# BaileyMeche/FM-ReturnPrediction

Hardware: AMD Instinct MI355X
Metric: firm-month rows/sec (and % HBM roofline) for full FM pass at 1/2/4/8 MI355X (higher is better)
Workload: dtype f64; 1 GPU; C3+C4 full pass per GPU: 600 months x 5000 firms x 15 chars; winsorize 1/99 -> NYSE universes -> M1/M2/M3 x 3 universes + Fig-1 x 2 -> NW(4) -> rolling 120/60 -> lagged-rolling forecasts + predictive-slope FM; months_per_gpu=600, firms=5000, chars=15, problems_per_month=11, global_months=600, seed=1, parallelism=month-sharded x1

## Files before the change

fm-returnprediction_amd/csrc/fm_solve.hip:

```cpp
#include <math.h>

#include <type_traits>

#include "fm_common.h"

FM_PROBE_BUFFER(solve)

namespace fm {
namespace {

constexpr int VT = 256;
constexpr int VNW = VT / WAVE;
constexpr int MAXB_LDS = 8192;
constexpr int64_t SCAN_GRID = 1024;
constexpr double CHOL_REL = 1e-9;
constexpr double EIG_REL = 1e-12;
constexpr double REFIT_REL = 1e-6;

template <int MD>
struct WaveScratch {
    double A[MD * MD];
    double V[MD * MD];
    double sxy[MD], sdiag[MD], mu[MD], b[MD];
};

template <int MD>
__device__ void jacobi_pinv(double* A, double* V, int K, const double* sxy, const double* mur, double* b) {
    for (int i = 0; i < K; ++i)
        for (int j = 0; j < K; ++j) V[i * MD + j] = i == j ? 1.0 : 0.0;
    double frob = 0.0;
    for (int i = 0; i < K; ++i)
        for (int j = 0; j < K; ++j) frob += A[i * MD + j] * A[i * MD + j];
    for (int sweep = 0; sweep < 80; ++sweep) {
        double off = 0.0;
        for (int p = 0; p < K; ++p)
            for (int q = p + 1; q < K; ++q) off += A[p * MD + q] * A[p * MD + q];
        if (off <= 1e-34 * frob) break;
        for (int p = 0; p < K; ++p) {
            for (int q = p + 1; q < K; ++q) {
                const double apq = A[p * MD + q];
                if (apq == 0.0) continue;
                const double theta = (A[q * MD + q] - A[p * MD + p]) / (2.0 * apq);
                const double t = (theta >= 0.0 ? 1.0 : -1.0) / (fabs(theta) + sqrt(theta * theta + 1.0));
                const double c = 1.0 / sqrt(t * t + 1.0), s = t * c;
                for (int k = 0; k < K; ++k) {
                    const double akp = A[k * MD + p], akq = A[k * MD + q];
                    A[k * MD + p] = c * akp - s * akq;
                    A[k * MD + q] = s * akp + c * akq;
                }
                for (int k = 0; k < K; ++k) {
                    const double apk = A[p * MD + k], aqk = A[q * MD + k];
                    A[p * MD + k] = c * apk - s * aqk;
                    A[q * MD + k] = s * apk + c * aqk;
                }
                A[p * MD + q] = 0.0;
                A[q * MD + p] = 0.0;
                for (int k = 0; k < K; ++k) {
                    const double vkp = V[k * MD + p], vkq = V[k * MD + q];
                    V[k * MD + p] = c * vkp - s * vkq;
                    V[k * MD + q] = s * vkp + c * vkq;
                }
            }
        }
    }
    double lmax = 0.0;
    for (int i = 0; i < K; ++i) lmax = fmax(lmax, fabs(A[i * MD + i]));
    for (int j = 0; j < K; ++j) b[j] = 0.0;
    for (int i = 0; i < K; ++i) {
        const double l = A[i * MD + i];
        if (!(l > EIG_REL * lmax)) continue;
        double proj = 0.0;
        for (int k = 0; k < K; ++k) proj += V[k * MD + i] * sxy[k];
        proj /= l;
        for (int j = 0; j < K; ++j) b[j] += proj * V[j * MD + i];
    }
    double b0 = mur[K], den = 1.0;
    for (int j = 0; j < K; ++j) b0 -= b[j] * mur[j];
    for (int i = 0; i < K; ++i) {
        if (A[i * MD + i] > EIG_REL * lmax) continue;
        double wi = 0.0;
        for (int k = 0; k < K; ++k) wi += V[k * MD + i] * mur[k];
        den += wi * wi;
    }
    if (!(den > 1.0) || !isfinite(b0)) return;
    for (int i = 0; i < K; ++i) {
        if (A[i * MD + i] > EIG_REL * lmax) continue;
        double wi = 0.0;
        for (int k = 0; k < K; ++k) wi += V[k * MD + i] * mur[k];
        const double t = b0 * wi / den;
        for (int j = 0; j < K; ++j) b[j] += t * V[j * MD + i];
    }
}

__device__ __forceinline__ double readlane_f64(double v, int l) {
    return __longlong_as_double((long long)readlane_u64((uint64_t)__double_as_longlong(v), l));
}

template <int NT>
__device__ __forceinline__ void sum_partials(const double* partial, int c0, int c1, int n, double* bs) {
    constexpr int BCH = 8;
    const int tid = threadIdx.x;
    for (int e0 = tid; e0 < n; e0 += NT * BCH) {
        double acc[BCH];
#pragma unroll
        for (int k = 0; k < BCH; ++k) acc[k] = 0.0;
        for (int c = c0; c < c1; ++c) {
            const double* pc = partial + (int64_t)c * n;
#pragma unroll
            for (int k = 0; k < BCH; ++k) {
                const int e = e0 + k * NT;
                acc[k] += pc[e < n ? e : n - 1];
            }
        }
#pragma unroll
        for (int k = 0; k < BCH; ++k) {
            const int e = e0 + k * NT;
            if (e < n) bs[e] = acc[k];
        }
    }
}

template <int MD>
__global__ __launch_bounds__(VT) void solve_kernel(fm_solve_args a) {
    extern __shared__ double bs[];
    __shared__ WaveScratch<MD> ws_all[VNW];
    const int s = blockIdx.x;
    const int tid = threadIdx.x, lane = tid & (WAVE - 1);
    const int w = __builtin_amdgcn_readfirstlane(tid / WAVE);
    const int zw = a.zw, zz = zw * (zw + 1) / 2;
    const int nl = a.nlevels, npat = a.npatterns, nb = npat * nl;
    const int c0 = a.seg_chunk_off[s], c1 = a.seg_chunk_off[s + 1];
    sum_partials<VT>(a.partial, c0, c1, nb * zz, bs);
    __syncthreads();
    for (int e = tid; e < npat * zz; e += VT) {
        const int pid = e / zz, f = e - pid * zz;
        double* b0 = bs + (int64_t)pid * nl * zz + f;
        double run = b0[(nl - 1) * zz];
        for (int l = nl - 2; l >= 0; --l) {
            run += b0[l * zz];
            b0[l * zz] = run;
        }
    }
    __syncthreads();
    WaveScratch<MD>& ws = ws_all[w];
    const int rs = a.pmax + 2;
    constexpr int PKW = MD * (MD + 1) / 2;
    constexpr int EPL = (PKW + WAVE - 1) / WAVE;
    for (int p = w; p < a.nprob; p += VNW) {
        const int m = a.prob_model[p], u = a.prob_level[p], nz = a.prob_nz[p];
        const int* zi = a.prob_z + p * 32;
        const int K = nz - 2, K1 = K + 1;
        int off[EPL], dst[EPL], dsw[EPL];
        double acc[EPL];
#pragma unroll
        for (int t = 0; t < EPL; ++t) {
            const int e = lane + WAVE * t;
            int i = 0, rem = e;
            while (i < nz && rem >= nz - i) {
                rem -= nz - i;
                ++i;
            }
            const bool in = i < nz;
            const int j = in ? i + rem : 0;
            const int zr = in ? zi[i] : 0, zc = in ? zi[j] : 0;
            const int r = zr < zc ? zr : zc, c = zr < zc ? zc : zr;
            off[t] = in ? r * zw - (r * (r - 1)) / 2 + (c - r) : 0;
            dst[t] = in ? i * MD + j : -1;
            dsw[t] = in ? j * MD + i : -1;
            acc[t] = 0.0;
        }
        for (int q = 0; q < npat; ++q) {
            if (!((a.pattern_models[q] >> m) & 1u)) continue;
            const double* bq = bs + (q * nl + u) * zz;
#pragma unroll
            for (int t = 0; t < EPL; ++t) acc[t] += bq[off[t]];
        }
#pragma unroll
        for (int t = 0; t < EPL; ++t)
            if (dst[t] >= 0) {
                ws.V[dst[t]] = acc[t];
                ws.V[dsw[t]] = acc[t];
            }
        wave_sync();
        const double* Gp = ws.V;
        const int zl = lane < K1 ? zi[1 + lane] : 0;
        const int li = lane < K1 ? 1 + lane : 0;
        const double n = Gp[0];
        const double g0 = lane < K1 ? Gp[li] : 0.0;
        const double gdiag = lane < K1 ? Gp[li * MD + li] : 0.0;
        const int64_t ro = ((int64_t)s * a.nprob + p) * rs;
        uint32_t st = 0;
        if (__ballot(lane < K && isinf(gdiag)) != 0) st |= FM_ST_INF_IN_X;
        if (__ballot(lane == K && isinf(gdiag)) != 0) st |= FM_ST_INF_IN_Y;
        if (a.gram_flags) st |= a.gram_flags[(int64_t)s * a.nmodels + m] & (FM_ST_INF_IN_X | FM_ST_INF_IN_Y);
        if (!(n >= (double)(K + 1))) {
            for (int k = lane; k < rs; k += WAVE) a.rec[ro + k] = k == a.pmax + 1 ? n : NAN;
            if (lane == 0) a.status[(int64_t)s * a.nprob + p] = FM_ST_SKIPPED;
            continue;
        }
        double row[MD];
        double sii = 0.0, sxy = 0.0;
#pragma unroll
        for (int j = 0; j < MD; ++j) {
            row[j] = 0.0;
            if (j < K1) {
                const double v = lane < K1 ? Gp[li * MD + 1 + j] - g0 * Gp[1 + j] / n : 0.0;
                row[j] = v;
                if (j == lane) sii = v;
                if (j == K) sxy = v;
            }
        }
        const double mu = g0 / n;
        if (a.moments) {
            double* mo = a.moments + ((int64_t)s * a.nprob + p) * a.mom_stride;
            if (lane == 0) mo[0] = n;
            if (lane < K1) {
                mo[1 + lane] = mu;
#pragma unroll
                for (int j = 0; j < MD; ++j)
                    if (j < K1) mo[1 + K1 + lane * K1 + j] = row[j];
            }
        }
        if ((a.prob_flags[p] & 1) != 0) {
            if (__ballot(lane < K && !(sii > 1e-10 * gdiag)) != 0) st |= FM_ST_CONST_SUSPECT;
        }
        const double syy = readlane_f64(sii, K);
        bool ok = true;
#pragma unroll
        for (int k = 0; k < MD - 1; ++k) {
            if (ok && k < K) {
                const double orig = readlane_f64(sii, k);
                const double piv = readlane_f64(row[k], k);
                if (!(piv > REFIT_REL * orig)) st |= FM_ST_REFIT;
                if (!(orig > 0.0) || !(piv > CHOL_REL * orig)) {
                    ok = false;
                } else {
                    const double lkk = sqrt(piv);
                    const double rinv = 1.0 / lkk;
                    const double lik = row[k] * rinv;
#pragma unroll
                    for (int j = k + 1; j < MD; ++j) {
                        if (j <= K) {
                            const double sj = readlane_f64(row[j], k) * rinv;
                            row[j] -= lik * sj;
                        }
                    }
                    row[k] = lane == k ? lkk : lik;
                }
            }
        }
        double bi = 0.0;
        if (ok) {
            double* T = ws.A;
#pragma unroll
            for (int j = 0; j < MD; ++j)
                if (lane < K1) T[lane * MD + j] = row[j];
            wave_sync();
            double col[MD];
#pragma unroll
            for (int r = 0; r < MD; ++r) col[r] = lane < MD ? T[r * MD + (lane & (MD - 1))] : 0.0;
            double t = lane < K ? T[K * MD + lane] : 0.0;
#pragma unroll
            for (int j = MD - 2; j >= 0; --j) {
                if (j < K) {
                    const double bj = readlane_f64(t, j) / readlane_f64(col[j], j);
                    if (lane == j) t = bj;
                    else if (lane < j) t -= col[j] * bj;
                }
            }
            bi = lane < K ? t : 0.0;
            wave_sync();
        } else {
            st |= FM_ST_RANK_DEF | FM_ST_REFIT;
#pragma unroll
            for (int j = 0; j < MD; ++j)
                if (j < K && lane < K) ws.A[lane * MD + j] = Gp[li * MD + 1 + j] - g0 * Gp[1 + j] / n;
            if (lane < K) ws.sxy[lane] = sxy;
            if (lane < K1) ws.mu[lane] = mu + (a.add_back ? a.add_back[(int64_t)(zl - 1) * a.nseg + s] : 0.0);
            wave_sync();
            if (lane == 0) jacobi_pinv<MD>(ws.A, ws.V, K, ws.sxy, ws.mu, ws.b);
            wave_sync();
            bi = lane < K ? ws.b[lane] : 0.0;
            wave_sync();
        }
        double t_sxy = lane < K ? bi * sxy : 0.0;
        double t_mu = lane < K ? bi * mu : 0.0;
        double t_ab = 0.0;
        if (a.add_back && lane < K) t_ab = bi * a.add_back[(int64_t)(zl - 1) * a.nseg + s];
        t_sxy = wave_sum(t_sxy);
        t_mu = wave_sum(t_mu);
        t_ab = wave_sum(t_ab);
        const double r2 = 1.0 - (syy - t_sxy) / syy;
        double icpt = readlane_f64(mu, K) - t_mu;
        if (a.add_back) icpt += a.add_back[(int64_t)(zi[K + 1] - 1) * a.nseg + s] - t_ab;
        const double bsh = __shfl(bi, lane > 0 ? lane - 1 : 0, WAVE);
        for (int k = lane; k < rs; k += WAVE) {
            double v = NAN;
            if (k == 0) v = icpt;
            else if (k <= K) v = bsh;
            else if (k == a.pmax) v = r2;
            else if (k == a.pmax + 1) v = n;
            a.rec[ro + k] = v;
        }
        if (lane == 0) a.status[(int64_t)s * a.nprob + p] = st | FM_ST_FITTED;
    }
}

template <class CA>
struct FixCtx {
    CA cols; int64_t stride; const int64_t* seg_off; int nseg;
    const double *lo, *hi;
    const double *shift, *inv_scale, *add_back;
    const uint8_t* level;
    int nprob; const int32_t *prob_level, *prob_z, *prob_nz;
    const double* moments; int mom_stride;
    int pmax; double* rec; uint32_t* status;
    int check_const;
};

template <class CA>
__host__ __device__ __forceinline__ FixCtx<CA> fix_ctx(const fm_solve_args& a, CA cols) {
    FixCtx<CA> fx{};
    fx.check_const = a.fix_check_const;
    fx.cols = cols, fx.stride = a.fix_stride, fx.seg_off = a.fix_seg_off, fx.nseg = a.nseg;
    fx.lo = a.fix_lo, fx.hi = a.fix_hi;
    fx.shift = a.fix_shift, fx.inv_scale = a.fix_inv_scale, fx.add_back = a.add_back;
    fx.level = a.fix_level;
    fx.nprob = a.nprob, fx.prob_level = a.prob_level, fx.prob_z = a.prob_z, fx.prob_nz = a.prob_nz;
    fx.moments = a.moments, fx.mom_stride = a.mom_stride;
    fx.pmax = a.pmax, fx.rec = a.rec, fx.status = a.status;
    return fx;
}

template <int NT = VT, class CA = F64Cols>
__device__ __forceinline__ void const_pair(int s, int p, uint64_t* red, const FixCtx<CA>& fx) {
    const int nz = fx.prob_nz[p], K = nz - 2, u = fx.prob_level[p];
    const int* zi = fx.prob_z + p * 32;
    const int64_t r0 = fx.seg_off[s], r1 = fx.seg_off[s + 1];
    bool any_const = false;
    for (int j = 0; j < K; ++j) {
        const int cx = zi[1 + j] - 1;
        uint64_t kmin = SENT, kmax = 0;
        bool allnz = true;
        for (int64_t r = r0 + threadIdx.x; r < r1; r += NT) {
            if (fx.level && (int)fx.level[r] < u) continue;
            bool ok = true;
            double xv = 0.0;
            for (int q = 1; q < nz; ++q) {
                const int c = zi[q] - 1;
                double x = fx.cols[(int64_t)c * fx.stride + r];
                if (fx.lo) {
                    const double l = fx.lo[(int64_t)c * fx.nseg + s], h = fx.hi[(int64_t)c * fx.nseg + s];
                    if (x < l) x = l;
                    if (x > h) x = h;
                }
                if (isnan(x)) ok = false;
                if (c == cx) xv = x;
            }
            if (!ok) continue;
            const uint64_t k = dkey(xv == 0.0 ? 0.0 : xv);
            kmin = k < kmin ? k : kmin;
            kmax = k > kmax ? k : kmax;
            if (xv == 0.0) allnz = false;
        }
        kmin = block_min_u64<NT / WAVE>(kmin, red);
        kmax = block_max_u64<NT / WAVE>(kmax, red);
        const int nzr = block_sum<NT / WAVE>(allnz ? 0 : 1, (int*)red);
        if (kmin != SENT && kmin == kmax && nzr == 0) any_const = true;
    }
    if (threadIdx.x == 0 && any_const) fx.status[(int64_t)s * fx.nprob + p] |= FM_ST_CONST_COL;
}

struct InfySmem {
    double Lm[32 * 32];
    double mu[32], xb[32];
    unsigned bits[32];
    int okf;
};

template <int NT = VT, int NC = 32, class CA = F64Cols>
__device__ __forceinline__ void infy_pair(int s, int p, InfySmem& sm, const FixCtx<CA>& fx) {
    double* Lm = sm.Lm;
    double* mu = sm.mu;
    double* xb = sm.xb;
    unsigned* bits = sm.bits;
    int& okf = sm.okf;
    const int nz = fx.prob_nz[p], K = nz - 2, K1 = K + 1, u = fx.prob_level[p];
    const int* zi = fx.prob_z + p * 32;
    const double* mo = fx.moments + ((int64_t)s * fx.nprob + p) * fx.mom_stride;
    const double n = mo[0];
    for (int e = threadIdx.x; e < K * K; e += NT) Lm[(e / K) * 32 + e % K] = mo[1 + K1 + (e / K) * K1 + e % K];
    if (threadIdx.x < K1) mu[threadIdx.x] = mo[1 + threadIdx.x];
    if (threadIdx.x < 32) bits[threadIdx.x] = 0u;
    __syncthreads();
    if (threadIdx.x < K) {
        const int c = zi[1 + threadIdx.x] - 1;
        xb[threadIdx.x] = mu[threadIdx.x] + (fx.add_back ? fx.add_back[(int64_t)c * fx.nseg + s] : 0.0);
    }
    if (threadIdx.x == 0) {
        int ok = 1;
        for (int k = 0; k < K && ok; ++k) {
            double d = Lm[k * 32 + k];
            for (int j = 0; j < k; ++j) d -= Lm[k * 32 + j] * Lm[k * 32 + j];
            if (!(d > 0.0)) { ok = 0; break; }
            d = sqrt(d);
            Lm[k * 32 + k] = d;
            for (int i = k + 1; i < K; ++i) {
                double t = Lm[i * 32 + k];
                for (int j = 0; j < k; ++j) t -= Lm[i * 32 + j] * Lm[k * 32 + j];
                Lm[i * 32 + k] = t / d;
            }
        }
        okf = ok;
    }
    __syncthreads();
    if (!okf) return;
    const int64_t r0 = fx.seg_off[s], r1 = fx.seg_off[s + 1];
    if constexpr (NC <= 16) {
        for (int64_t r = r0 + threadIdx.x; r < r1; r += NT) {
            if (fx.level && (int)fx.level[r] < u) continue;
            int zo = 0;
            asm volatile("" : "+v"(zo));
            double d[NC];
            double y = 0.0;
            bool valid = true;
#pragma unroll
            for (int q = 1; q <= NC; ++q) {
                if (q < nz) {
                    const int c = zi[q] - 1;
                    double x = fx.cols[(int64_t)c * fx.stride + r];
                    if (fx.lo) {
                        const double l = fx.lo[(int64_t)c * fx.nseg + s], h = fx.hi[(int64_t)c * fx.nseg + s];
                        if (x < l) x = l;
                        if (x > h) x = h;
                    }
                    if (isnan(x)) valid = false;
                    if (q == nz - 1) {
                        y = x;
                    } else {
                        if (fx.shift) x -= fx.shift[(int64_t)c * fx.nseg + s];
                        if (fx.inv_scale) x *= fx.inv_scale[(int64_t)c * fx.nseg + s];
                        d[q - 1] = x - mu[q - 1 + zo];
                    }
                }
            }
            if (!valid || !isinf(y)) continue;
#pragma unroll
            for (int i = 0; i < NC; ++i) {
                if (i < K) {
                    double t = d[i];
#pragma unroll
                    for (int j = 0; j < i; ++j) t -= Lm[i * 32 + j + zo] * d[j];
                    d[i] = t / Lm[i * 32 + i + zo];
                }
            }
#pragma unroll
            for (int i = NC - 1; i >= 0; --i) {
                if (i < K) {
                    double t = d[i];
#pragma unroll
                    for (int j = i + 1; j < NC; ++j)
                        if (j < K) t -= Lm[j * 32 + i + zo] * d[j];
                    d[i] = t / Lm[i * 32 + i + zo];
                }
            }
            double c0 = 1.0 / n;
#pragma unroll
            for (int j = 0; j < NC; ++j)
                if (j < K) c0 -= xb[j + zo] * d[j];
#pragma unroll
            for (int j = 0; j <= NC; ++j) {
                if (j <= K) {
                    const double term = (j == 0 ? c0 : d[j == 0 ? 0 : j - 1]) * y;
                    const unsigned b = isnan(term) ? 4u : (term > 0.0 ? 1u : 2u);
                    atomicOr(&bits[j], b);
                }
            }
        }
    } else
    for (int64_t r = r0 + threadIdx.x; r < r1; r += NT) {
        if (fx.level && (int)fx.level[r] < u) continue;
        double v[32];
        bool valid = true;
        for (int q = 1; q < nz; ++q) {
            const int c = zi[q] - 1;
            double x = fx.cols[(int64_t)c * fx.stride + r];
            if (fx.lo) {
                const double l = fx.lo[(int64_t)c * fx.nseg + s], h = fx.hi[(int64_t)c * fx.nseg + s];
                if (x < l) x = l;
                if (x > h) x = h;
            }
            if (isnan(x)) valid = false;
            v[q - 1] = x;
        }
        if (!valid || !isinf(v[K])) continue;
        const double y = v[K];
        double d[32];
        for (int j = 0; j < K; ++j) {
            const int c = zi[1 + j] - 1;
            double x = v[j];
            if (fx.shift) x -= fx.shift[(int64_t)c * fx.nseg + s];
            if (fx.inv_scale) x *= fx.inv_scale[(int64_t)c * fx.nseg + s];
            d[j] = x - mu[j];
        }
        for (int i = 0; i < K; ++i) {
            double t = d[i];
            for (int j = 0; j < i; ++j) t -= Lm[i * 32 + j] * d[j];
            d[i] = t / Lm[i * 32 + i];
        }
        for (int i = K - 1; i >= 0; --i) {
            double t = d[i];
            for (int j = i + 1; j < K; ++j) t -= Lm[j * 32 + i] * d[j];
            d[i] = t / Lm[i * 32 + i];
        }
        double c0 = 1.0 / n;
        for (int j = 0; j < K; ++j) c0 -= xb[j] * d[j];
        for (int j = 0; j <= K; ++j) {
            const double term = (j == 0 ? c0 : d[j - 1]) * y;
            const unsigned b = isnan(term) ? 4u : (term > 0.0 ? 1u : 2u);
            atomicOr(&bits[j], b);
        }
    }
    __syncthreads();
    const int64_t ro = ((int64_t)s * fx.nprob + p) * (fx.pmax + 2);
    if (threadIdx.x <= K) {
        const unsigned b = bits[threadIdx.x];
        if (b != 0u) {
            double val = NAN;
            if (!(b & 4u) && b != 3u) val = (b & 1u) ? INFINITY : -INFINITY;
            fx.rec[ro + threadIdx.x] = val;
        }
    }
    if (threadIdx.x == 0) fx.rec[ro + fx.pmax] = NAN;
}

constexpr double SVD_REL = 1e-13;

__device__ __forceinline__ double wave_sum_dpp(double v) {
    v += xor_lanes_f64(v, 1);
    v += xor_lanes_f64(v, 2);
    v += xor_lanes_f64(v, 4);
    v += xor_lanes_f64(v, 8);
    v += xor_lanes_f64(v, 16);
    v += xor_lanes_f64(v, 32);
    return v;
}

template <int NC, int NW = VNW>
struct RefitSmem {
    double R[NW][NC][NC + 1];
    double Ac[NC][NC + 1];
    double Vc[NC][NC + 1];
    double bv[NC];
};

template <int NC>
__device__ __forceinline__ void hh_absorb(double (&a)[NC], double (*R)[NC + 1], int nzc) {
    const int lane = lane_id();
    static_for<0, NC>([&](auto kc) {
        constexpr int k = decltype(kc)::value;
        if (k < nzc) {
            const double ss = wave_sum_dpp(a[k] * a[k]);
            if (ss != 0.0) {
                const double alpha = R[k][k];
                const double nrm = sqrt(alpha * alpha + ss);
                const double beta = alpha > 0.0 ? -nrm : nrm;
                const double v0 = alpha - beta;
                const double tau = -v0 / beta;
                const double vl = a[k] / v0;
                double w[NC];
                static_for<k + 1, NC>([&](auto jc) {
                    constexpr int j = decltype(jc)::value;
                    w[j] = vl * a[j];
                });
                static_for<k + 1, NC>([&](auto jc) {
                    constexpr int j = decltype(jc)::value;
                    w[j] = wave_sum_dpp(w[j]) + R[k][j];
                });
                static_for<k + 1, NC>([&](auto jc) {
                    constexpr int j = decltype(jc)::value;
                    a[j] -= (tau * w[j]) * vl;
                });
                __builtin_amdgcn_fence(__ATOMIC_RELEASE, "wavefront");
                __builtin_amdgcn_wave_barrier();
                __builtin_amdgcn_fence(__ATOMIC_ACQUIRE, "wavefront");
                if (lane == 0) {
                    R[k][k] = beta;
                    static_for<k + 1, NC>([&](auto jc) {
                        constexpr int j = decltype(jc)::value;
                        R[k][j] -= tau * w[j];
                    });
                }
                __builtin_amdgcn_fence(__ATOMIC_RELEASE, "wavefront");
                __builtin_amdgcn_wave_barrier();
                __builtin_amdgcn_fence(__ATOMIC_ACQUIRE, "wavefront");
                a[k] = 0.0;
            }
        }
    });
}

template <int NC, int NT = VT, class CA = F64Cols>
__device__ void refit_pair(int s, int p, RefitSmem<NC, NT / WAVE>& sm, const FixCtx<CA>& fx) {
    const int tid = threadIdx.x, lane = tid & (WAVE - 1), w = tid / WAVE;
    const int nz = fx.prob_nz[p], P = nz - 1, u = fx.prob_level[p];
    const int* zi = fx.prob_z + p * 32;
    constexpr int NW = NT / WAVE;
    for (int e = tid; e < NW * NC * (NC + 1); e += NT) (&sm.R[0][0][0])[e] = 0.0;
    __syncthreads();
    int zc[NC];
    static_for<0, NC>([&](auto qc) {
        constexpr int q = decltype(qc)::value;
        zc[q] = (q >= 1 && q < nz) ? zi[q] - 1 : 0;
    });
    const int64_t r0 = fx.seg_off[s], r1 = fx.seg_off[s + 1];
    for (int64_t base = r0 + (int64_t)w * WAVE; base < r1; base += NT) {
        const int64_t r = base + lane;
        bool valid = r < r1 && !(fx.level && (int)fx.level[r] < u);
        double a[NC];
        static_for<0, NC>([&](auto qc) {
            constexpr int q = decltype(qc)::value;
            double v = 0.0;
            if constexpr (q == 0) {
                v = 1.0;
            } else {
                if (valid && q < nz) {
                    const int c = zc[q];
                    double x = fx.cols[(int64_t)c * fx.stride + r];
                    if (fx.lo) {
                        const double l = fx.lo[(int64_t)c * fx.nseg + s], h = fx.hi[(int64_t)c * fx.nseg + s];
                        if (x < l) x = l;
                        if (x > h) x = h;
                    }
                    if (fx.inv_scale) {
                        x = (x - fx.shift[(int64_t)c * fx.nseg + s]) * fx.inv_scale[(int64_t)c * fx.nseg + s];
                        if (fx.add_back) x += fx.add_back[(int64_t)c * fx.nseg + s];
                    }
                    if (isnan(x)) valid = false;
                    v = x;
                }
            }
            a[q] = v;
        });
        static_for<0, NC>([&](auto qc) {
            constexpr int q = decltype(qc)::value;
            if (!valid) a[q] = 0.0;
        });
        hh_absorb<NC>(a, sm.R[w], nz);
    }
    __syncthreads();
    if (w == 0) {
        for (int o = 1; o < NW; ++o) {
            double a[NC];
            static_for<0, NC>([&](auto jc) {
                constexpr int j = decltype(jc)::value;
                a[j] = (lane < NC && j >= lane) ? sm.R[o][lane < NC ? lane : 0][j] : 0.0;
            });
            hh_absorb<NC>(a, sm.R[0], nz);
        }
        double (*R)[NC + 1] = sm.R[0];
        const bool li = lane < P;
        const int lr = li ? lane : 0;
        if (li)
            for (int j = 0; j < P; ++j) {
                sm.Ac[j][lane] = j >= lane ? R[lane][j] : 0.0;
                sm.Vc[j][lane] = j == lane ? 1.0 : 0.0;
            }
        __builtin_amdgcn_fence(__ATOMIC_RELEASE, "wavefront");
        __builtin_amdgcn_wave_barrier();
        __builtin_amdgcn_fence(__ATOMIC_ACQUIRE, "wavefront");
        for (int sweep = 0; sweep < 60; ++sweep) {
            bool rotated = false;
            for (int pc = 0; pc < P - 1; ++pc) {
                for (int qc = pc + 1; qc < P; ++qc) {
                    const double ap = li ? sm.Ac[pc][lr] : 0.0, aq = li ? sm.Ac[qc][lr] : 0.0;
                    const double al = wave_sum_dpp(ap * ap);
                    const double be = wave_sum_dpp(aq * aq);
                    const double ga = wave_sum_dpp(ap * aq);
                    if (!(fabs(ga) > 1e-15 * sqrt(al * be))) continue;
                    rotated = true;
                    const double zeta = (be - al) / (2.0 * ga);
                    const double t = fabs(zeta) > 1e150
                                         ? 0.5 / zeta
                                         : (zeta >= 0.0 ? 1.0 : -1.0) / (fabs(zeta) + sqrt(1.0 + zeta * zeta));
                    const double c = 1.0 / sqrt(1.0 + t * t), sn = c * t;
                    const double vp = li ? sm.Vc[pc][lr] : 0.0, vq = li ? sm.Vc[qc][lr] : 0.0;
                    if (li) {
                        sm.Ac[pc][lane] = c * ap - sn * aq;
                        sm.Ac[qc][lane] = sn * ap + c * aq;
                        sm.Vc[pc][lane] = c * vp - sn * vq;
                        sm.Vc[qc][lane] = sn * vp + c * vq;
                    }
                    __builtin_amdgcn_fence(__ATOMIC_RELEASE, "wavefront");
                    __builtin_amdgcn_wave_barrier();
                    __builtin_amdgcn_fence(__ATOMIC_ACQUIRE, "wavefront");
                }
            }
            if (!rotated) break;
        }
        const double ry = li ? R[lane][P] : 0.0;
        const double rho = R[P][P];
        double smax = 0.0;
        for (int j = 0; j < P; ++j) smax = fmax(smax, wave_sum_dpp(li ? sm.Ac[j][lr] * sm.Ac[j][lr] : 0.0));
        smax = sqrt(smax);
        double bi = 0.0;
        bool cut = false;
        for (int j = 0; j < P; ++j) {
            const double aj = li ? sm.Ac[j][lr] : 0.0;
            const double s2 = wave_sum_dpp(aj * aj);
            if (!(sqrt(s2) > SVD_REL * smax)) {
                cut = true;
                continue;
            }
            const double cj = wave_sum_dpp(aj * ry) / s2;
            if (li) bi += sm.Vc[j][lane] * cj;
        }
        if (li) sm.bv[lane] = bi;
        __builtin_amdgcn_fence(__ATOMIC_RELEASE, "wavefront");
        __builtin_amdgcn_wave_barrier();
        __builtin_amdgcn_fence(__ATOMIC_ACQUIRE, "wavefront");
        double fit = 0.0;
        if (li)
            for (int j = lane; j < P; ++j) fit += R[lane][j] * sm.bv[j];
        const double e = li ? ry - fit : 0.0;
        const double ssr = wave_sum_dpp(e * e) + rho * rho;
        const double tss = wave_sum_dpp((li && lane >= 1) ? ry * ry : 0.0) + rho * rho;
        const int64_t ro = ((int64_t)s * fx.nprob + p) * (fx.pmax + 2);
        if (li) fx.rec[ro + lane] = bi;
        if (lane == 0) {
            fx.rec[ro + fx.pmax] = 1.0 - ssr / tss;
            const uint32_t st = fx.status[(int64_t)s * fx.nprob + p];
            fx.status[(int64_t)s * fx.nprob + p] = (st & ~FM_ST_RANK_DEF) | (cut ? FM_ST_RANK_DEF : 0u);
        }
    }
}

template <int NC, int NT>
union FixSmem {
    InfySmem infy;
    RefitSmem<NC, NT / WAVE> refit;
    uint64_t red[NT / WAVE];
};
inline __device__ bool fix_wanted(uint32_t st, int check_const) {
    return (check_const && (st & FM_ST_CONST_SUSPECT)) ||
           ((st & FM_ST_FITTED) && (st & (FM_ST_INF_IN_Y | FM_ST_REFIT)));
}
template <int NC, int NT, class CA>
__device__ __forceinline__ void fix_one(int s, int p, uint32_t st, FixSmem<NC, NT>& sm, const FixCtx<CA>& fx) {
    if (fx.check_const && (st & FM_ST_CONST_SUSPECT)) {
        const_pair<NT>(s, p, sm.red, fx);
        __syncthreads();
    }
    if (!(st & FM_ST_FITTED)) return;
    if (st & FM_ST_INF_IN_Y) {
        infy_pair<NT, NC>(s, p, sm.infy, fx);
    } else if ((st & FM_ST_REFIT) && !(st & FM_ST_INF_IN_X) && fx.prob_nz[p] <= NC) {
        refit_pair<NC, NT>(s, p, sm.refit, fx);
    } else {
        return;
    }
    __syncthreads();
}


__device__ __forceinline__ double rsq_nr(double x) {
    double y = __builtin_amdgcn_rsq(x);
    const double h = 0.5 * x;
    y = y * fma(-h * y, y, 1.5);
    y = y * fma(-h * y, y, 1.5);
    return y;
}

template <int L>
__device__ __forceinline__ int rowbc_i(int v) {
    return __builtin_amdgcn_mov_dpp(v, 0x150 + L, 0xF, 0xF, true);
}
template <int L>
__device__ __forceinline__ double rowbc(double v) {
    const uint64_t b = (uint64_t)__double_as_longlong(v);
    const uint32_t lo = (uint32_t)rowbc_i<L>((int)(uint32_t)b), hi = (uint32_t)rowbc_i<L>((int)(uint32_t)(b >> 32));
    return __longlong_as_double((long long)(((uint64_t)hi << 32) | lo));
}
__device__ __forceinline__ double rowsum(double v) { return row16_sum(v); }

constexpr int G16 = 16;

constexpr int S16T = 192;
constexpr int S16W = S16T / WAVE;
constexpr int S16_MAXP = 32;
__global__ __launch_bounds__(S16T, 3) void solve16_kernel(fm_solve_args a) {
    extern __shared__ double bs[];
    constexpr int TT = G16 * (G16 + 1);
    static_assert(sizeof(WaveScratch<16>) <= 4 * TT * sizeof(double), "scratch union");
    __shared__ double wsc[S16W][4 * TT];
    static_assert(sizeof(FixSmem<G16, S16T>) <= sizeof(wsc), "solve16's inline fix-ups reuse its per-wave scratch");
    const int s = blockIdx.x;
    const int tid = threadIdx.x, lane = tid & (WAVE - 1);
    const int w = __builtin_amdgcn_readfirstlane(tid / WAVE);
    constexpr int zw = 16, zz = 136;
    const int nl = a.nlevels, npat = a.npatterns, nb = npat * nl;
    __shared__ int t_model[S16_MAXP], t_level[S16_MAXP], t_nz[S16_MAXP], t_flags[S16_MAXP];
    __shared__ int t_slot[S16_MAXP];
    __shared__ uint32_t t_st[S16_MAXP];
    __shared__ uint8_t t_z[S16_MAXP][32];
    __shared__ uint32_t t_pat[64];
    __shared__ double t_ab[32];
    for (int e = tid; e < a.nprob * 32; e += S16T) t_z[e >> 5][e & 31] = (uint8_t)a.prob_z[e];
    if (tid < a.nprob) {
        t_model[tid] = a.prob_model[tid];
        t_level[tid] = a.prob_level[tid];
        const int nzp = a.prob_nz[tid];
        t_nz[tid] = nzp;
        t_flags[tid] = a.prob_flags[tid];
        int rank = 0;
        for (int q = 0; q < a.nprob; ++q) {
            const int nzq = a.prob_nz[q];
            rank += (nzq > nzp || (nzq == nzp && q < tid)) ? 1 : 0;
        }
        t_slot[rank] = tid;
    }
    if (tid < npat) t_pat[tid] = a.pattern_models[tid];
    if (a.add_back && tid >= 64 && tid < 96) {
        const int c = tid - 64;
        t_ab[c] = c < a.ab_ncols ? a.add_back[(int64_t)c * a.nseg + s] : 0.0;
    }
    FM_PROBE_AT(solve, 0);
    const int c0 = a.seg_chunk_off[s], c1 = a.seg_chunk_off[s + 1];
    sum_partials<S16T>(a.partial, c0, c1, nb * zz, bs);
    __syncthreads();
    FM_PROBE_AT(solve, 1);
    for (int e = tid; e < npat * zz; e += S16T) {
        const int pid = e / zz, f = e - pid * zz;
        double* b0 = bs + (int64_t)pid * nl * zz + f;
        double run = b0[(nl - 1) * zz];
        for (int l = nl - 2; l >= 0; --l) {
            run += b0[l * zz];
            b0[l * zz] = run;
        }
    }
    __syncthreads();
    FM_PROBE_AT(solve, 2);
    const int g = lane >> 4, i = lane & 15;
    const int rs = a.pmax + 2;
    double* T = wsc[w] + g * TT;
    for (int p0 = w * 4; p0 < a.nprob; p0 += S16W * 4) {
        const int p = p0 + g;
        const bool live = p < a.nprob;
        const int pp = t_slot[live ? p : p0];
        const int m = t_model[pp], u = t_level[pp], nz = t_nz[pp];
        const int K = nz - 2, K1 = K + 1;
        const int kw = __builtin_amdgcn_readfirstlane(K);
        const int zi = i < nz ? t_z[pp][i] : 0;
        auto gram_row = [&](double (&G)[G16]) {
            int off[G16];
            static_for<0, G16>([&](auto jc) {
                constexpr int j = decltype(jc)::value;
                const int zj = rowbc_i<j>(zi);
                const int r = zi < zj ? zi : zj, c = zi < zj ? zj : zi;
                off[j] = r * zw - (r * (r - 1)) / 2 + (c - r);
            });
#pragma unroll
            for (int j = 0; j < G16; ++j) G[j] = 0.0;
            for (int q = 0; q < npat; ++q) {
                if (!((t_pat[q] >> m) & 1u)) continue;
                const double* bq = bs + (q * nl + u) * zz;
#pragma unroll
                for (int j = 0; j < G16; ++j)
                    if (j < kw + 2) G[j] += bq[off[j]];
            }
        };
        double G[G16];
        gram_row(G);
        const double n = rowbc<0>(G[0]);
        const double ninv = 1.0 / n;
        const bool srow = i >= 1 && i <= K1;
        double row[G16];
        double sii = 0.0, sxy = 0.0, gdiag = 0.0;
        static_for<0, G16>([&](auto jc) {
            constexpr int j = decltype(jc)::value;
            gdiag = i == j ? G[j] : gdiag;
            if constexpr (j + 1 < G16) {
                if (j > kw) {
                    row[j] = 0.0;
                    return;
                }
                const double g0j = rowbc<0>(G[j + 1]);
                const double v = srow && j < K1 ? G[j + 1] - G[0] * g0j * ninv : 0.0;
                row[j] = v;
                sii = i == j + 1 ? v : sii;
                sxy = j == K ? v : sxy;
            } else {
                row[j] = 0.0;
            }
        });
        FM_PROBE_AT(solve, 4);
        const double mu = G[0] * ninv;
        const uint64_t gm = 0xFFFFull << (16 * g);
        uint32_t st = 0;
        if ((__ballot(i >= 1 && i <= K && isinf(gdiag)) & gm) != 0) st |= FM_ST_INF_IN_X;
        if ((__ballot(i == K1 && isinf(gdiag)) & gm) != 0) st |= FM_ST_INF_IN_Y;
        const int64_t ro = ((int64_t)s * a.nprob + pp) * rs;
        const bool skip = !(n >= (double)(K + 1));
        if (live && skip) {
            for (int k = i; k < rs; k += G16) a.rec[ro + k] = k == a.pmax + 1 ? n : NAN;
            if (i == 0) a.status[(int64_t)s * a.nprob + pp] = t_st[pp] = FM_ST_SKIPPED;
        }
        const bool act0 = live && !skip;
        if (act0 && a.moments) {
            double* mo = a.moments + ((int64_t)s * a.nprob + pp) * a.mom_stride;
            if (i == 0) mo[0] = n;
            if (srow) {
                mo[i] = mu;
#pragma unroll
                for (int c = 0; c < G16 - 1; ++c)
                    if (c < K1) mo[1 + K1 + c * K1 + (i - 1)] = row[c];
            }
        }
        if (act0 && (t_flags[pp] & 1) != 0) {
            if ((__ballot(i >= 1 && i <= K && !(sii > 1e-10 * gdiag)) & gm) != 0) st |= FM_ST_CONST_SUSPECT;
        }
        FM_PROBE_AT(solve, 5);
        bool ok = act0, illc = false;
        double dinv = 0.0;
        static_for<0, G16 - 1>([&](auto kc) {
            constexpr int k = decltype(kc)::value;
            if (k >= kw) return;
            const bool act = ok && k < K;
            const double orig = rowbc<k + 1>(sii);
            const double piv = rowbc<k + 1>(row[k]);
            if (act && !(piv > REFIT_REL * orig)) illc = true;
            const bool bad = act && (!(orig > 0.0) || !(piv > CHOL_REL * orig));
            if (bad) ok = false;
            const bool go = act && !bad;
            const double rinv = rsq_nr(piv);
            const double lkk = piv * rinv;
            const double lik = row[k] * rinv;
            static_for<k + 1, G16>([&](auto jc) {
                constexpr int j = decltype(jc)::value;
                if (j > kw) return;
                const double sj = rowbc<k + 1>(row[j]) * rinv;
                row[j] = row[j] - lik * sj;
            });
            row[k] = go ? (i == k + 1 ? lkk : lik) : row[k];
            dinv = i == k + 1 ? rinv : dinv;
        });
        FM_PROBE_AT(solve, 6);
        const bool rank_def = act0 && !ok;
        if (srow) {
#pragma unroll
            for (int c = 0; c < G16; ++c) T[(i - 1) * (G16 + 1) + c] = row[c];
        }
        __builtin_amdgcn_fence(__ATOMIC_RELEASE, "wavefront");
        __builtin_amdgcn_wave_barrier();
        __builtin_amdgcn_fence(__ATOMIC_ACQUIRE, "wavefront");
        double col[G16];
        const int rr = i >= 1 ? i - 1 : 0;
#pragma unroll
        for (int c = 0; c < G16 - 1; ++c) col[c] = T[c * (G16 + 1) + rr];
        col[G16 - 1] = 0.0;
        double t = (i >= 1 && i <= K) ? T[K * (G16 + 1) + rr] : 0.0;
        static_for<0, G16 - 1>([&](auto jc) {
            constexpr int j = 14 - decltype(jc)::value;
            if (j >= kw) return;
            const double bj = rowbc<j + 1>(t) * rowbc<j + 1>(dinv);
            if (ok && j < K) {
                if (i == j + 1) t = bj;
                else if (i >= 1 && i - 1 < j) t -= col[j] * bj;
            }
        });
        __builtin_amdgcn_fence(__ATOMIC_RELEASE, "wavefront");
        __builtin_amdgcn_wave_barrier();
        __builtin_amdgcn_fence(__ATOMIC_ACQUIRE, "wavefront");
        FM_PROBE_AT(solve, 7);
        double bi = (ok && i >= 1 && i <= K) ? t : 0.0;
        const uint64_t rd = __ballot(rank_def && i == 0);
        double G2[G16];
        if (rd) gram_row(G2);
        for (uint64_t q = rd; q; q &= q - 1) {
            const int gq = __builtin_ctzll(q) >> 4;
            WaveScratch<16>& J = *reinterpret_cast<WaveScratch<16>*>(wsc[w]);
            const int Kq = __shfl(K, gq * 16, WAVE);
            const double (&G)[G16] = G2;
            {
                double g0c[G16 - 1];
#pragma unroll
                for (int c = 0; c < G16 - 1; ++c) g0c[c] = __shfl(G[c + 1], gq * 16, WAVE);
                const double nq = __shfl(n, gq * 16, WAVE);
                if (g == gq && i >= 1 && i <= Kq) {
#pragma unroll
                    for (int c = 0; c < G16 - 1; ++c)
                        if (c < Kq) J.A[(i - 1) * 16 + c] = G[c + 1] - G[0] * g0c[c] / nq;
                    J.sxy[i - 1] = sxy;
                }
                if (g == gq && i >= 1 && i <= Kq + 1)
                    J.mu[i - 1] = mu + (a.add_back ? t_ab[zi - 1] : 0.0);
            }
            wave_sync();
            if (lane == 0) jacobi_pinv<16>(J.A, J.V, Kq, J.sxy, J.mu, J.b);
            wave_sync();
            if (g == gq && i >= 1 && i <= Kq) bi = J.b[i - 1];
            wave_sync();
        }
        if (rank_def) st |= FM_ST_RANK_DEF;
        if (illc) st |= FM_ST_REFIT;
        const bool xl = i >= 1 && i <= K;
        double t_sxy = xl ? bi * sxy : 0.0;
        double t_mu = xl ? bi * mu : 0.0;
        double t_abx = 0.0;
        if (a.add_back && xl && act0) t_abx = bi * t_ab[zi - 1];
        t_sxy = rowsum(t_sxy);
        t_mu = rowsum(t_mu);
        t_abx = rowsum(t_abx);
        const double syy = __shfl(sii, g * 16 + (K1 < 16 ? K1 : 15), WAVE);
        const double muy = __shfl(mu, g * 16 + (K1 < 16 ? K1 : 15), WAVE);
        const double r2 = 1.0 - (syy - t_sxy) / syy;
        double icpt = muy - t_mu;
        if (a.add_back && act0) {
            const int zy = t_z[pp][K + 1];
            icpt += t_ab[zy - 1] - t_abx;
        }
        if (act0) {
            for (int k = i; k < rs; k += G16) {
                double v = NAN;
                if (k == 0) v = icpt;
                else if (k <= K) v = k == i ? bi : NAN;
                else if (k == a.pmax) v = r2;
                else if (k == a.pmax + 1) v = n;
                a.rec[ro + k] = v;
            }
            if (i == 0) a.status[(int64_t)s * a.nprob + pp] = t_st[pp] = st | FM_ST_FITTED;
        }
    }
    FM_PROBE_AT(solve, 3);
    auto fix_all = [&](auto cols) {
        __syncthreads();
        const FixCtx<decltype(cols)> fx = fix_ctx(a, cols);
        for (int q = 0; q < a.nprob; ++q) {
            const uint32_t st = t_st[q];
            if (!fix_wanted(st, fx.check_const)) continue;
            fix_one<G16, S16T>(s, q, st, *reinterpret_cast<FixSmem<G16, S16T>*>(&wsc[0][0]), fx);
        }
    };
    if (a.fix_cols != nullptr) fix_all(F64Cols{a.fix_cols});
    else if (a.fix_hi_plane != nullptr) fix_all(PlaneCols{a.fix_hi_plane, (int64_t)(a.fix_lo_plane - a.fix_hi_plane)});
}

template <int NC>
__global__ __launch_bounds__(VT) void fixup_kernel(FixCtx<F64Cols> fx) {
    __shared__ FixSmem<NC, VT> sm;
    __shared__ int flagged[VT];
    __shared__ int nflag;
    const int total = fx.nseg * fx.nprob;
    const int tid = threadIdx.x;
    FM_PROBE_AT(solve, 4);
    for (int base = blockIdx.x * VT; base < total; base += gridDim.x * VT) {
        if (tid == 0) nflag = 0;
        __syncthreads();
        {
            const int e = base + tid;
            if (e < total && fix_wanted(fx.status[e], fx.check_const)) flagged[atomicAdd(&nflag, 1)] = e;
        }
        __syncthreads();
        const int nf = nflag;
        for (int f = 0; f < nf; ++f) {
            const int sp = flagged[f];
            const int s = sp / fx.nprob, p = sp - s * fx.nprob;
            fix_one<NC, VT>(s, p, fx.status[sp], sm, fx);
        }
        __syncthreads();
    }
    FM_PROBE_AT(solve, 5);
}

int check_fix_args(const fm_solve_args& a, const char* who) {
    FM_REQUIRE(a.fix_seg_off != nullptr, "%s: fix_seg_off is NULL", who);
    FM_REQUIRE(a.moments != nullptr, "%s: the fix-ups need moments", who);
    FM_REQUIRE((a.fix_lo == nullptr) == (a.fix_hi == nullptr), "%s: fix_lo and fix_hi go together", who);
    FM_REQUIRE(a.fix_inv_scale == nullptr || a.fix_shift != nullptr, "%s: fix_inv_scale needs fix_shift", who);
    FM_REQUIRE(a.pmax >= 2 && a.pmax <= 32, "%s: pmax must be 2..32", who);
    return FM_OK;
}

}
}

extern "C" int fm_solve(const fm_solve_args* args, void* stream) {
    using namespace fm;
    FM_REQUIRE(args != nullptr, "fm_solve: null args");
    const fm_solve_args& a = *args;
    FM_REQUIRE(a.partial && a.seg_chunk_off && a.pattern_models && a.prob_model && a.prob_level &&
                   a.prob_z && a.prob_nz && a.prob_flags && a.rec && a.status,
               "fm_solve: null pointer");
    FM_REQUIRE(a.zw == 16 || a.zw == 32, "fm_solve: zw must be 16 or 32");
    FM_REQUIRE(a.npatterns * a.nlevels * (a.zw * (a.zw + 1) / 2) <= MAXB_LDS,
               "fm_solve: %d buckets of a %d-wide Gram exceed the LDS budget", a.npatterns * a.nlevels, a.zw);
    FM_REQUIRE(a.pmax >= 2 && a.pmax <= 32, "fm_solve: pmax must be 2..32");
    FM_REQUIRE(a.moments == nullptr || a.mom_stride > 0, "fm_solve: bad mom_stride");
    FM_REQUIRE(a.add_back == nullptr || (a.ab_ncols >= 1 && a.ab_ncols <= FM_MAX_COLS),
               "fm_solve: add_back needs ab_ncols in 1..%d", FM_MAX_COLS);
    FM_REQUIRE(a.zw == 32 || a.nprob <= S16_MAXP, "fm_solve: at most %d problems per group", S16_MAXP);
    FM_REQUIRE((a.fix_hi_plane == nullptr) == (a.fix_lo_plane == nullptr),
               "fm_solve: fix_hi_plane and fix_lo_plane go together");
    if (a.fix_cols != nullptr || a.fix_hi_plane != nullptr) {
        FM_REQUIRE(a.zw == 16 && a.pmax + 1 <= 16, "fm_solve: inline fix-ups need zw 16 and pmax <= 15");
        if (const int rc = check_fix_args(a, "fm_solve")) return rc;
    }
    if (a.nseg == 0 || a.nprob == 0) return FM_OK;
    const size_t dyn = (size_t)a.npatterns * a.nlevels * (a.zw * (a.zw + 1) / 2) * sizeof(double);
    const int rc = a.zw == 16 ? raise_dynamic_lds<solve16_kernel>(MAXB_LDS * sizeof(double), "fm_solve")
                              : raise_dynamic_lds<solve_kernel<32>>(MAXB_LDS * sizeof(double), "fm_solve");
    if (rc != FM_OK) return rc;
    if (a.zw == 16)
        hipLaunchKernelGGL(solve16_kernel, dim3(a.nseg), dim3(S16T), dyn, (hipStream_t)stream, a);
    else
        hipLaunchKernelGGL(solve_kernel<32>, dim3(a.nseg), dim3(VT), dyn, (hipStream_t)stream, a);
    FM_CHECK_LAUNCH("fm_solve");
    return FM_OK;
}

extern "C" int fm_solve_fixup(const fm_solve_args* args, void* stream) {
    using namespace fm;
    FM_REQUIRE(args != nullptr, "fm_solve_fixup: null args");
    const fm_solve_args& a = *args;
    FM_REQUIRE(a.fix_hi_plane == nullptr && a.fix_lo_plane == nullptr, "fm_solve_fixup: FP64 columns only (a plane is set)");
    FM_REQUIRE(a.fix_cols && a.prob_level && a.prob_z && a.prob_nz && a.rec && a.status, "fm_solve_fixup: null pointer");
    if (const int rc = check_fix_args(a, "fm_solve_fixup")) return rc;
    const int64_t work = (int64_t)a.nseg * a.nprob;
    if (work == 0) return FM_OK;
    const int64_t ranges = (work + VT - 1) / VT;
    const int grid = (int)(ranges < SCAN_GRID ? ranges : SCAN_GRID);
    const FixCtx<F64Cols> fx = fix_ctx(a, F64Cols{a.fix_cols});
    if (a.pmax + 1 <= 16)
        hipLaunchKernelGGL(fixup_kernel<16>, dim3(grid), dim3(VT), 0, (hipStream_t)stream, fx);
    else
        hipLaunchKernelGGL(fixup_kernel<32>, dim3(grid), dim3(VT), 0, (hipStream_t)stream, fx);
    FM_CHECK_LAUNCH("fm_solve_fixup");
    return FM_OK;
}
```

Measured before the change: 12.76 billion firm-month rows/s.

## Specialize solve16 Cholesky by regressor-count width and add tiny-scale rescaling

Moves the per-problem Gram build, Cholesky and back-substitution of solve16 into a templated factor16 instantiated for widths 3, 5, 7 and 14. A wave-uniform dispatch on K picks the instance, so small problems skip unused columns and need fewer registers. It also writes L rows to LDS inside the factor loop, drops the per-element kw guards, and batches bucket loads before accumulating them. Separately, it adds exponent rescaling in rsq_nr and column scaling in refit for tiny sums of squares, plus a flag that sends such columns to refit; these are numerical-robustness changes that add a little work.

```diff
diff --git a/fm-returnprediction_amd/csrc/fm_solve.hip b/fm-returnprediction_amd/csrc/fm_solve.hip
--- a/fm-returnprediction_amd/csrc/fm_solve.hip
+++ b/fm-returnprediction_amd/csrc/fm_solve.hip
@@ -535,6 +535,7 @@
 }
 
 constexpr double SVD_REL = 1e-13;
+constexpr double TINY_SS = 0x1p-1000;
 
 __device__ __forceinline__ double wave_sum_dpp(double v) {
     v += xor_lanes_f64(v, 1);
@@ -607,6 +608,15 @@
     const int* zi = fx.prob_z + p * 32;
     constexpr int NW = NT / WAVE;
     for (int e = tid; e < NW * NC * (NC + 1); e += NT) (&sm.R[0][0][0])[e] = 0.0;
+    if (tid < NC) {
+        double f = 1.0;
+        if (tid >= 1 && tid <= P - 1) {
+            const int K1 = P;
+            const double sd = fx.moments[((int64_t)s * fx.nprob + p) * fx.mom_stride + 1 + K1 + (tid - 1) * K1 + (tid - 1)];
+            if (sd > 0.0 && sd < TINY_SS) f = __builtin_ldexp(1.0, -ilogb(sd) / 2);
+        }
+        sm.bv[tid] = f;
+    }
     __syncthreads();
     int zc[NC];
     static_for<0, NC>([&](auto qc) {
@@ -637,7 +647,7 @@
                         if (fx.add_back) x += fx.add_back[(int64_t)c * fx.nseg + s];
                     }
                     if (isnan(x)) valid = false;
-                    v = x;
+                    v = x * sm.bv[q];
                 }
             }
             a[q] = v;
@@ -715,6 +725,10 @@
             const double cj = wave_sum_dpp(aj * ry) / s2;
             if (li) bi += sm.Vc[j][lane] * cj;
         }
+        const double cs = li ? sm.bv[lane] : 1.0;
+        __builtin_amdgcn_fence(__ATOMIC_RELEASE, "wavefront");
+        __builtin_amdgcn_wave_barrier();
+        __builtin_amdgcn_fence(__ATOMIC_ACQUIRE, "wavefront");
         if (li) sm.bv[lane] = bi;
         __builtin_amdgcn_fence(__ATOMIC_RELEASE, "wavefront");
         __builtin_amdgcn_wave_barrier();
@@ -726,7 +740,7 @@
         const double ssr = wave_sum_dpp(e * e) + rho * rho;
         const double tss = wave_sum_dpp((li && lane >= 1) ? ry * ry : 0.0) + rho * rho;
         const int64_t ro = ((int64_t)s * fx.nprob + p) * (fx.pmax + 2);
-        if (li) fx.rec[ro + lane] = bi;
+        if (li) fx.rec[ro + lane] = bi * cs;
         if (lane == 0) {
             fx.rec[ro + fx.pmax] = 1.0 - ssr / tss;
             const uint32_t st = fx.status[(int64_t)s * fx.nprob + p];
@@ -764,11 +778,13 @@
 
 
 __device__ __forceinline__ double rsq_nr(double x) {
-    double y = __builtin_amdgcn_rsq(x);
-    const double h = 0.5 * x;
+    const int e = x < 0x1p-767 ? 768 : 0;
+    const double xs = __builtin_ldexp(x, e);
+    double y = __builtin_amdgcn_rsq(xs);
+    const double h = 0.5 * xs;
     y = y * fma(-h * y, y, 1.5);
     y = y * fma(-h * y, y, 1.5);
-    return y;
+    return __builtin_ldexp(y, e >> 1);
 }
 
 template <int L>
@@ -784,20 +800,169 @@
 __device__ __forceinline__ double rowsum(double v) { return row16_sum(v); }
 
 constexpr int G16 = 16;
+constexpr int Z16 = G16 * (G16 + 1) / 2;
+constexpr int TT = G16 * (G16 + 1);
+
+template <int NJ>
+__device__ __forceinline__ void gram_offsets(int zi, int (&off)[NJ]) {
+    static_for<0, NJ>([&](auto jc) {
+        constexpr int j = decltype(jc)::value;
+        const int zj = rowbc_i<j>(zi);
+        const int r = zi < zj ? zi : zj, c = zi < zj ? zj : zi;
+        off[j] = r * G16 - (r * (r - 1)) / 2 + (c - r);
+    });
+}
+
+struct Buckets16 {
+    const double* bs;
+    const uint32_t* pat;
+    int npat, nl;
+};
+
+template <int NJ>
+__device__ __forceinline__ void gram_row(const Buckets16& B, int m, int u, int zi, double (&G)[NJ]) {
+    int off[NJ];
+    gram_offsets<NJ>(zi, off);
+#pragma unroll
+    for (int j = 0; j < NJ; ++j) G[j] = 0.0;
+    for (int q = 0; q < B.npat; ++q) {
+        if (!((B.pat[q] >> m) & 1u)) continue;
+        const double* bq = B.bs + (q * B.nl + u) * Z16;
+        double v[NJ];
+#pragma unroll
+        for (int j = 0; j < NJ; ++j) v[j] = bq[off[j]];
+        __builtin_amdgcn_sched_barrier(0);
+#pragma unroll
+        for (int j = 0; j < NJ; ++j) G[j] += v[j];
+    }
+}
+
+struct Slot16 {
+    int s, pp, m, u, K, zi;
+    bool live;
+    int flags;
+};
+struct Fact16 {
+    double n, mu, sii, sxy, t;
+    bool act0, ok, illc;
+    uint32_t st;
+};
+
+template <int KW>
+__device__ __forceinline__ Fact16 factor16(const fm_solve_args& a, const Slot16& q, const Buckets16& B, double* T,
+                                           uint32_t* t_st) {
+    static_assert(KW >= 1 && KW <= G16 - 2, "factor16: 1..14 regressors");
+    const int lane = lane_id(), g = lane >> 4, i = lane & 15;
+    const int K = q.K, K1 = K + 1;
+    double G[KW + 2];
+    gram_row<KW + 2>(B, q.m, q.u, q.zi, G);
+    const double n = rowbc<0>(G[0]);
+    const double ninv = 1.0 / n;
+    const bool srow = i >= 1 && i <= K1;
+    double row[KW + 1];
+    double sii = 0.0, sxy = 0.0, gdiag = 0.0;
+    static_for<0, KW + 2>([&](auto jc) {
+        constexpr int j = decltype(jc)::value;
+        gdiag = i == j ? G[j] : gdiag;
+    });
+    static_for<0, KW + 1>([&](auto jc) {
+        constexpr int j = decltype(jc)::value;
+        const double g0j = rowbc<0>(G[j + 1]);
+        const double c = G[j + 1] - G[0] * g0j * ninv;
+        const double v = (srow & (j < K1)) ? c : 0.0;
+        row[j] = v;
+        sii = i == j + 1 ? v : sii;
+        sxy = j == K ? v : sxy;
+    });
+    FM_PROBE_AT(solve, 4);
+    const double mu = G[0] * ninv;
+    const uint64_t gm = 0xFFFFull << (16 * g);
+    uint32_t st = 0;
+    if ((__ballot(i >= 1 && i <= K && isinf(gdiag)) & gm) != 0) st |= FM_ST_INF_IN_X;
+    if ((__ballot(i == K1 && isinf(gdiag)) & gm) != 0) st |= FM_ST_INF_IN_Y;
+    const int rs = a.pmax + 2;
+    const int64_t ro = ((int64_t)q.s * a.nprob + q.pp) * rs;
+    const bool skip = !(n >= (double)(K + 1));
+    if (q.live && skip) {
+        for (int k = i; k < rs; k += G16) a.rec[ro + k] = k == a.pmax + 1 ? n : NAN;
+        if (i == 0) a.status[(int64_t)q.s * a.nprob + q.pp] = t_st[q.pp] = FM_ST_SKIPPED;
+    }
+    const bool act0 = q.live && !skip;
+    if (act0 && a.moments) {
+        double* mo = a.moments + ((int64_t)q.s * a.nprob + q.pp) * a.mom_stride;
+        if (i == 0) mo[0] = n;
+        if (srow) {
+            mo[i] = mu;
+#pragma unroll
+            for (int c = 0; c < KW + 1; ++c)
+                if (c < K1) mo[1 + K1 + c * K1 + (i - 1)] = row[c];
+        }
+    }
+    if (act0 && (q.flags & 1) != 0) {
+        if ((__ballot(i >= 1 && i <= K && !(sii > 1e-10 * gdiag)) & gm) != 0) st |= FM_ST_CONST_SUSPECT;
+    }
+    FM_PROBE_AT(solve, 5);
+    bool ok = act0;
+    int illc = (act0 && (__ballot(i >= 1 && i <= K && sii > 0.0 && sii < TINY_SS) & gm) != 0) ? 1 : 0;
+    const int tr = i >= 1 ? i - 1 : G16 - 1;
+    double dinv = 0.0;
+    static_for<0, KW>([&](auto kc) {
+        constexpr int k = decltype(kc)::value;
+        const bool act = ok & (k < K);
+        const double orig = rowbc<k + 1>(sii);
+        const double piv = rowbc<k + 1>(row[k]);
+        illc |= (act & !(piv > REFIT_REL * orig)) ? 1 : 0;
+        asm volatile("" : "+v"(illc));
+        const bool bad = act & (!(orig > 0.0) | !(piv > CHOL_REL * orig));
+        ok = ok & !bad;
+        const bool go = act & !bad;
+        const double rinv = rsq_nr(piv);
+        const double lkk = piv * rinv;
+        const double lik = row[k] * rinv;
+        static_for<k + 1, KW + 1>([&](auto jc) {
+            constexpr int j = decltype(jc)::value;
+            const double sj = rowbc<k + 1>(row[j]) * rinv;
+            row[j] = row[j] - lik * sj;
+        });
+        row[k] = go ? (i == k + 1 ? lkk : lik) : row[k];
+        dinv = i == k + 1 ? rinv : dinv;
+        T[tr * (G16 + 1) + k] = row[k];
+    });
+    FM_PROBE_AT(solve, 6);
+    __builtin_amdgcn_fence(__ATOMIC_RELEASE, "wavefront");
+    __builtin_amdgcn_wave_barrier();
+    __builtin_amdgcn_fence(__ATOMIC_ACQUIRE, "wavefront");
+    double col[KW];
+    const int rr = i >= 1 ? i - 1 : 0;
+#pragma unroll
+    for (int c = 0; c < KW; ++c) col[c] = T[c * (G16 + 1) + rr];
+    double t = (i >= 1 && i <= K) ? T[K * (G16 + 1) + rr] : 0.0;
+    static_for<0, KW>([&](auto jc) {
+        constexpr int j = KW - 1 - decltype(jc)::value;
+        const double bj = rowbc<j + 1>(t) * rowbc<j + 1>(dinv);
+        const double tm = t - col[j] * bj;
+        const double tn = i == j + 1 ? bj : (((i >= 1) & (i - 1 < j)) ? tm : t);
+        t = (ok & (j < K)) ? tn : t;
+    });
+    __builtin_amdgcn_fence(__ATOMIC_RELEASE, "wavefront");
+    __builtin_amdgcn_wave_barrier();
+    __builtin_amdgcn_fence(__ATOMIC_ACQUIRE, "wavefront");
+    FM_PROBE_AT(solve, 7);
+    return Fact16{n, mu, sii, sxy, t, act0, ok, illc != 0, st};
+}
 
 constexpr int S16T = 192;
 constexpr int S16W = S16T / WAVE;
 constexpr int S16_MAXP = 32;
 __global__ __launch_bounds__(S16T, 3) void solve16_kernel(fm_solve_args a) {
     extern __shared__ double bs[];
-    constexpr int TT = G16 * (G16 + 1);
     static_assert(sizeof(WaveScratch<16>) <= 4 * TT * sizeof(double), "scratch union");
     __shared__ double wsc[S16W][4 * TT];
     static_assert(sizeof(FixSmem<G16, S16T>) <= sizeof(wsc), "solve16's inline fix-ups reuse its per-wave scratch");
     const int s = blockIdx.x;
     const int tid = threadIdx.x, lane = tid & (WAVE - 1);
     const int w = __builtin_amdgcn_readfirstlane(tid / WAVE);
-    constexpr int zw = 16, zz = 136;
+    constexpr int zz = Z16;
     const int nl = a.nlevels, npat = a.npatterns, nb = npat * nl;
     __shared__ int t_model[S16_MAXP], t_level[S16_MAXP], t_nz[S16_MAXP], t_flags[S16_MAXP];
     __shared__ int t_slot[S16_MAXP];
@@ -839,143 +1004,35 @@
         }
     }
     __syncthreads();
-    FM_PROBE_AT(solve, 2);
+    const Buckets16 B{bs, t_pat, npat, nl};
     const int g = lane >> 4, i = lane & 15;
     const int rs = a.pmax + 2;
     double* T = wsc[w] + g * TT;
+    FM_PROBE_AT(solve, 2);
     for (int p0 = w * 4; p0 < a.nprob; p0 += S16W * 4) {
         const int p = p0 + g;
         const bool live = p < a.nprob;
         const int pp = t_slot[live ? p : p0];
         const int m = t_model[pp], u = t_level[pp], nz = t_nz[pp];
-        const int K = nz - 2, K1 = K + 1;
+        const int K = nz - 2;
+        const int zi = i < nz ? t_z[pp][i] : 0;
+        const Slot16 sl{s, pp, m, u, K, zi, live, t_flags[pp]};
         const int kw = __builtin_amdgcn_readfirstlane(K);
-        const int zi = i < nz ? t_z[pp][i] : 0;
-        auto gram_row = [&](double (&G)[G16]) {
-            int off[G16];
-            static_for<0, G16>([&](auto jc) {
-                constexpr int j = decltype(jc)::value;
-                const int zj = rowbc_i<j>(zi);
-                const int r = zi < zj ? zi : zj, c = zi < zj ? zj : zi;
-                off[j] = r * zw - (r * (r - 1)) / 2 + (c - r);
-            });
-#pragma unroll
-            for (int j = 0; j < G16; ++j) G[j] = 0.0;
-            for (int q = 0; q < npat; ++q) {
-                if (!((t_pat[q] >> m) & 1u)) continue;
-                const double* bq = bs + (q * nl + u) * zz;
-#pragma unroll
-                for (int j = 0; j < G16; ++j)
-                    if (j < kw + 2) G[j] += bq[off[j]];
-            }
-        };
-        double G[G16];
-        gram_row(G);
-        const double n = rowbc<0>(G[0]);
-        const double ninv = 1.0 / n;
-        const bool srow = i >= 1 && i <= K1;
-        double row[G16];
-        double sii = 0.0, sxy = 0.0, gdiag = 0.0;
-        static_for<0, G16>([&](auto jc) {
-            constexpr int j = decltype(jc)::value;
-            gdiag = i == j ? G[j] : gdiag;
-            if constexpr (j + 1 < G16) {
-                if (j > kw) {
-                    row[j] = 0.0;
-                    return;
-                }
-                const double g0j = rowbc<0>(G[j + 1]);
-                const double v = srow && j < K1 ? G[j + 1] - G[0] * g0j * ninv : 0.0;
-                row[j] = v;
-                sii = i == j + 1 ? v : sii;
-                sxy = j == K ? v : sxy;
-            } else {
-                row[j] = 0.0;
-            }
-        });
-        FM_PROBE_AT(solve, 4);
-        const double mu = G[0] * ninv;
-        const uint64_t gm = 0xFFFFull << (16 * g);
-        uint32_t st = 0;
-        if ((__ballot(i >= 1 && i <= K && isinf(gdiag)) & gm) != 0) st |= FM_ST_INF_IN_X;
-        if ((__ballot(i == K1 && isinf(gdiag)) & gm) != 0) st |= FM_ST_INF_IN_Y;
+        Fact16 F;
+        if (kw <= 3) F = factor16<3>(a, sl, B, T, t_st);
+        else if (kw <= 5) F = factor16<5>(a, sl, B, T, t_st);
+        else if (kw <= 7) F = factor16<7>(a, sl, B, T, t_st);
+        else F = factor16<14>(a, sl, B, T, t_st);
+        const double n = F.n, mu = F.mu, sii = F.sii, sxy = F.sxy;
+        const bool act0 = F.act0, ok = F.ok;
+        uint32_t st = F.st;
+        const int K1 = K + 1;
         const int64_t ro = ((int64_t)s * a.nprob + pp) * rs;
-        const bool skip = !(n >= (double)(K + 1));
-        if (live && skip) {
-            for (int k = i; k < rs; k += G16) a.rec[ro + k] = k == a.pmax + 1 ? n : NAN;
-            if (i == 0) a.status[(int64_t)s * a.nprob + pp] = t_st[pp] = FM_ST_SKIPPED;
-        }
-        const bool act0 = live && !skip;
-        if (act0 && a.moments) {
-            double* mo = a.moments + ((int64_t)s * a.nprob + pp) * a.mom_stride;
-            if (i == 0) mo[0] = n;
-            if (srow) {
-                mo[i] = mu;
-#pragma unroll
-                for (int c = 0; c < G16 - 1; ++c)
-                    if (c < K1) mo[1 + K1 + c * K1 + (i - 1)] = row[c];
-            }
-        }
-        if (act0 && (t_flags[pp] & 1) != 0) {
-            if ((__ballot(i >= 1 && i <= K && !(sii > 1e-10 * gdiag)) & gm) != 0) st |= FM_ST_CONST_SUSPECT;
-        }
-        FM_PROBE_AT(solve, 5);
-        bool ok = act0, illc = false;
-        double dinv = 0.0;
-        static_for<0, G16 - 1>([&](auto kc) {
-            constexpr int k = decltype(kc)::value;
-            if (k >= kw) return;
-            const bool act = ok && k < K;
-            const double orig = rowbc<k + 1>(sii);
-            const double piv = rowbc<k + 1>(row[k]);
-            if (act && !(piv > REFIT_REL * orig)) illc = true;
-            const bool bad = act && (!(orig > 0.0) || !(piv > CHOL_REL * orig));
-            if (bad) ok = false;
-            const bool go = act && !bad;
-            const double rinv = rsq_nr(piv);
-            const double lkk = piv * rinv;
-            const double lik = row[k] * rinv;
-            static_for<k + 1, G16>([&](auto jc) {
-                constexpr int j = decltype(jc)::value;
-                if (j > kw) return;
-                const double sj = rowbc<k + 1>(row[j]) * rinv;
-                row[j] = row[j] - lik * sj;
-            });
-            row[k] = go ? (i == k + 1 ? lkk : lik) : row[k];
-            dinv = i == k + 1 ? rinv : dinv;
-        });
-        FM_PROBE_AT(solve, 6);
         const bool rank_def = act0 && !ok;
-        if (srow) {
-#pragma unroll
-            for (int c = 0; c < G16; ++c) T[(i - 1) * (G16 + 1) + c] = row[c];
-        }
-        __builtin_amdgcn_fence(__ATOMIC_RELEASE, "wavefront");
-        __builtin_amdgcn_wave_barrier();
-        __builtin_amdgcn_fence(__ATOMIC_ACQUIRE, "wavefront");
-        double col[G16];
-        const int rr = i >= 1 ? i - 1 : 0;
-#pragma unroll
-        for (int c = 0; c < G16 - 1; ++c) col[c] = T[c * (G16 + 1) + rr];
-        col[G16 - 1] = 0.0;
-        double t = (i >= 1 && i <= K) ? T[K * (G16 + 1) + rr] : 0.0;
-        static_for<0, G16 - 1>([&](auto jc) {
-            constexpr int j = 14 - decltype(jc)::value;
-            if (j >= kw) return;
-            const double bj = rowbc<j + 1>(t) * rowbc<j + 1>(dinv);
-            if (ok && j < K) {
-                if (i == j + 1) t = bj;
-                else if (i >= 1 && i - 1 < j) t -= col[j] * bj;
-            }
-        });
-        __builtin_amdgcn_fence(__ATOMIC_RELEASE, "wavefront");
-        __builtin_amdgcn_wave_barrier();
-        __builtin_amdgcn_fence(__ATOMIC_ACQUIRE, "wavefront");
-        FM_PROBE_AT(solve, 7);
-        double bi = (ok && i >= 1 && i <= K) ? t : 0.0;
+        double bi = (ok && i >= 1 && i <= K) ? F.t : 0.0;
         const uint64_t rd = __ballot(rank_def && i == 0);
         double G2[G16];
-        if (rd) gram_row(G2);
+        if (rd) gram_row<G16>(B, m, u, zi, G2);
         for (uint64_t q = rd; q; q &= q - 1) {
             const int gq = __builtin_ctzll(q) >> 4;
             WaveScratch<16>& J = *reinterpret_cast<WaveScratch<16>*>(wsc[w]);
@@ -1002,7 +1059,7 @@
             wave_sync();
         }
         if (rank_def) st |= FM_ST_RANK_DEF;
-        if (illc) st |= FM_ST_REFIT;
+        if (F.illc) st |= FM_ST_REFIT;
         const bool xl = i >= 1 && i <= K;
         double t_sxy = xl ? bi * sxy : 0.0;
         double t_mu = xl ? bi * mu : 0.0;
```

New measurement: 12.94 billion firm-month rows/s (median of 6 runs). +1.4%, better.
